# damaggu/StableKeypoints

Measured on AMD Instinct MI355X. Metric: images/sec (token-opt step, 512², N=500 tokens), higher is better.
Workload: dtype f32

## Files before the change

stablekeypoints_amd/csrc/skp_conv.hip:

```cpp
#include <cstdlib>
#include <initializer_list>
#include <type_traits>

#include "skp_common.h"
#include "skp_gn.h"

using namespace skp;

#ifndef SKP_WINO_DEBUG
#define SKP_WINO_DEBUG 0
#endif
#ifndef SKP_WINO2_DEBUG
#define SKP_WINO2_DEBUG 0
#endif

namespace {

typedef float f32x4 __attribute__((ext_vector_type(4)));
typedef unsigned int u32x4 __attribute__((ext_vector_type(4)));

constexpr int kMT = 64;
constexpr int kNC = 32;
constexpr int kCK = 4;
constexpr int kP = 36;
// ... 329 lines not shown
  if (!(a.nsplit == 1 || a.ws))
    return (form & kStride2) ? "split-K needs a workspace of nsplit·B·K·(H/2)·(W/2) floats"
                             : "split-K needs a workspace of nsplit·B·K·H·W floats";
  if (!a.aligned) return "tensors must be 16-byte aligned";
  if (!(form & kHW32) && (long long)a.B * (a.H / 4) * (a.W / 4) > 0x7fffffffLL - kMT) return "too many tiles";
  if ((form & kOffsets32) && !((long long)a.B * a.C * a.H * a.W * 4 < 0x7fffffffLL))
    return "input larger than 2 GiB (32-bit buffer offsets)";
  return nullptr;
}
constexpr long long kMaxGrid = 0x7fffffffLL;

}

extern "C" int skp_wino_weights(const float* w, int K, int C, int flip, float* U, void* stream) {
  const char* err = weights_args_error(w, U, K, C);
  SKP_CHECK_ARG(!err, err);
  const long long n = (long long)K * C;
  hipLaunchKernelGGL(wino_weights_kernel<kP>, dim3((unsigned)((n + 255) / 256)), dim3(256), 0, as_stream(stream), w, K,
                     C, flip, U);
  SKP_LAUNCH_CHECK();
  return SKP_OK;
}

namespace {

__global__ void splitk_reduce_kernel(const float4* __restrict__ ws, int nsplit, long long n4, int K, int hw4,
                                     const float* __restrict__ bias, const float4* __restrict__ res,
                                     float4* __restrict__ y) {
  const long long i = blockIdx.x * (long long)blockDim.x + threadIdx.x;
  if (i >= n4) return;
  float4 v = ws[i];
  for (int s = 1; s < nsplit; ++s) {
    const float4 p = ws[(long long)s * n4 + i];
    v.x += p.x;
    v.y += p.y;
    v.z += p.z;
    v.w += p.w;
  }
  if (bias) {
    const float b = bias[(i / hw4) % K];
    v.x += b;
    v.y += b;
    v.z += b;
    v.w += b;
  }
  if (res) {
    const float4 r = res[i];
    v.x += r.x;
    v.y += r.y;
    v.z += r.z;
    v.w += r.w;
  }
  y[i] = v;
}

int splitk_reduce(const float* ws, int nsplit, int B, int K, int HW, const float* bias, const float* residual,
                  float* y, hipStream_t st) {
  const long long n4 = (long long)B * K * HW / 4;
  hipLaunchKernelGGL(splitk_reduce_kernel, dim3((unsigned)((n4 + 255) / 256)), dim3(256), 0, st,
                     reinterpret_cast<const float4*>(ws), nsplit, n4, K, HW / 4, bias,
                     reinterpret_cast<const float4*>(residual), reinterpret_cast<float4*>(y));
  SKP_LAUNCH_CHECK();
  return SKP_OK;
}

int wino_nt_flag(long long out_bytes, int nsplit) {
  if (nsplit > 1) return 0;
  return out_bytes >= (256LL << 20) ? 128 : 0;
}

template <int NEPI, class F>
auto with_epi(int epi, F&& f) {
  static_assert(NEPI == 2 || NEPI == 4, "bias only, or bias and residual");
  if constexpr (NEPI == 4) {
    if (epi == 2) return f(std::integral_constant<int, 2>{});
    if (epi == 3) return f(std::integral_constant<int, 3>{});
  }
  return epi == 1 ? f(std::integral_constant<int, 1>{}) : f(std::integral_constant<int, 0>{});
}

template <class Launch>
int conv_launch(const char* entry, const float* bias, const float* residual, float* y, float* ws, int nsplit, int B, int K,
                int hw, int dbg, bool nt, hipStream_t st, Launch&& launch) {
  const int epi = nsplit > 1 ? 0 : (bias ? 1 : 0) | (residual ? 2 : 0);
  launch(epi, nsplit > 1 ? ws : y, dbg | (nt ? wino_nt_flag((long long)B * K * hw * 4, nsplit) : 0));
  const hipError_t e = hipGetLastError();
  if (e != hipSuccess) {
    set_error(std::string(entry) + ": launch failed: " + hipGetErrorString(e));
    return SKP_ELAUNCH;
  }
  if (nsplit > 1) return splitk_reduce(ws, nsplit, B, K, hw, bias, residual, y, st);
  return SKP_OK;
}

}

extern "C" int skp_conv3x3_wino(const float* x, const float* U, const float* bias, const float* residual, float* y,
                                int B, int C, int K, int H, int W, int nsplit, float* ws, void* stream) {
  const ConvArgs a{x && U && y, all_aligned16({x, U, y, residual, ws}), ws, nullptr, B, C, K, H, W, nsplit, 1};
  const char* err = conv_args_error(kOffsets32, a);
  const int tw = W / 4, tpi = (H / 4) * tw;
  const long long ntiles = (long long)B * tpi;
  const bool wide = ntiles <= 32 && K % 64 == 0;
  const int mt = wide ? 32 : kMT;
  const int ntb = (int)((ntiles + mt - 1) / mt), nkb = K / (wide ? 64 : kNC);
  if (!err && (long long)ntb * nkb * nsplit > kMaxGrid) err = "grid too large";
  SKP_CHECK_ARG(!err, err);
  const long long ubytes = (long long)K * C * kP * 4;
  const int kb_major = ubytes > (2LL << 20);
  hipStream_t st = as_stream(stream);
  const dim3 grid((unsigned)(ntb * nkb * nsplit));
  return conv_launch(__func__, bias, residual, y, ws, nsplit, B, K, H * W, SKP_WINO_DEBUG, false, st,
                     [&](int epi, float* out, int dbg) {
                       const auto kernel = with_epi<4>(
                           epi, [&](auto E) { return wide ? wino_f4_kernel<E(), 32> : wino_f4_kernel<E(), 64>; });
                       hipLaunchKernelGGL(kernel, grid, dim3(kThreads), 0, st, x, U, bias, residual, out, B, C, K, H, W, tw,
                                          tpi, (int)ntiles, ntb, nkb, kb_major, C / nsplit, dbg);
                     });
}

namespace {
namespace w2 {

constexpr int kNC = 32;
constexpr int kCK = 4;
constexpr int kNW = 4;
template <int TXB>
struct GeoN;
template <>
struct GeoN<8> {
  static constexpr int NI = 1, RR = 18, RC = 10, CHF = 768;
};
template <>
struct GeoN<4> {
  static constexpr int NI = 2, RR = 18, RC = 6, CHF = 880;
};
template <int TXB>
struct GeoT : GeoN<TXB> {
  using GeoN<TXB>::NI;
  using GeoN<TXB>::RR;
  using GeoN<TXB>::RC;
  using GeoN<TXB>::CHF;
  static constexpr int RF = 4 * RC;
  static constexpr int RAWF = (4 * CHF + 255) / 256 * 256;
  static constexpr int RAW_INSTR = RAWF / 256;
  static_assert(NI * RR * RF <= CHF, "channel region");
};
constexpr int kUP = 40;
constexpr int kUF = kCK * kNC * kUP;
constexpr int kUInstr = kUF / 256;
constexpr unsigned kOOB = 0x80000000u;
constexpr int kVWF = 4 * 256 + 128;
constexpr int kVF = 4 * kVWF;
constexpr int kUP2 = 28;
constexpr int kUF2 = kCK * kNC * kUP2;
typedef unsigned int u32x2 __attribute__((ext_vector_type(2)));
static_assert(kUF % 256 == 0 && kUF2 % 256 == 0, "whole 1-KB chunks");
static_assert((3 * GeoT<8>::RAWF + 2 * kUF) * 4 <= 80 * 1024 && 2 * (GeoT<4>::RAWF + kUF) * 4 <= 80 * 1024,
              "rings of two workgroups per CU");

__device__ constexpr float kAt[4][6] = {{1.f, 1.f, 1.f, 1.f, 1.f, 0.f},
                                        {0.f, 1.f, -1.f, 0.5f, -2.f, 0.f},
                                        {0.f, 1.f, 1.f, 0.25f, 4.f, 0.f},
                                        {0.f, 1.f, -1.f, 0.125f, -8.f, 1.f}};

#define W2_VMCNT(n) __builtin_amdgcn_s_waitcnt(((n) & 15) | (((n) >> 4) << 14) | (7 << 4) | (15 << 8))

typedef float f2 __attribute__((ext_vector_type(2)));

template <typename T>
__device__ __forceinline__ void bt6_shared(T a0, T a1, T a2, T a3, T a4, T a5, T* y) {
  const T e = a4 - a2, f = a3 - a1, g = a2 + a3, h = a3 - a2;
  y[0] = __builtin_elementwise_fma((T)1.5f, f, (a0 + e) - a2);
  y[1] = __builtin_elementwise_fma((T)1.5f, g, e + f);
  y[2] = __builtin_elementwise_fma((T)1.5f, h, e - f);
  y[3] = __builtin_elementwise_fma((T)2.0f, f, e);
  y[4] = __builtin_elementwise_fma((T)-0.5f, f, e);
  y[5] = __builtin_elementwise_fma((T)1.5f, e, __builtin_elementwise_fma((T)-2.0f, f, a5 - a1));
}

template <int H, int RF>
__device__ __forceinline__ void half_transform_pk(const float* raw, float* a) {
  f2 t[3][3];
  f2 k0[3], k1[3], k2[3], k3[3];
#pragma unroll
  for (int r = 0; r < 6; ++r) {
    if (H == 1 && r == 0) continue;
    const f32x4 c0 = *reinterpret_cast<const f32x4*>(raw + r * RF);
    const f32x4 c1 = *reinterpret_cast<const f32x4*>(raw + r * RF + 4);
    const f32x4 c2 = *reinterpret_cast<const f32x4*>(raw + r * RF + 8);
    const f2 d[3] = {__builtin_shufflevector(c1, c1, 0, 1), __builtin_shufflevector(c1, c1, 2, 3),
                     __builtin_shufflevector(c0, c2, 3, 4)};
#pragma unroll
    for (int p = 0; p < 3; ++p) {
      if (H == 0) {
        if (r == 0) k0[p] = d[p];
        if (r == 1) { k1[p] = d[p]; k0[p] = __builtin_elementwise_fma((f2)-1.5f, d[p], k0[p]); }
        if (r == 2) { k2[p] = d[p]; k3[p] = __builtin_elementwise_fma((f2)1.5f, d[p], -k1[p]); }
        if (r == 3) { k1[p] = __builtin_elementwise_fma((f2)1.5f, d[p], -k2[p]); k3[p] = k3[p] + d[p]; }
        if (r == 4) {
          const f2 sv = k1[p] + d[p];
          t[0][p] = k0[p] + (sv - k2[p]);
          t[1][p] = sv + k3[p];
          t[2][p] = sv - k3[p];
        }
      } else {
        if (r == 1) k0[p] = d[p];
        if (r == 2) k1[p] = d[p];
        if (r == 3) { k2[p] = d[p] - k0[p]; k3[p] = __builtin_elementwise_fma((f2)-2.0f, k2[p], -k0[p]); }
        if (r == 4) {
          const f2 e = d[p] - k1[p];
          t[0][p] = __builtin_elementwise_fma((f2)2.0f, k2[p], e);
          t[1][p] = __builtin_elementwise_fma((f2)-0.5f, k2[p], e);
          k3[p] = __builtin_elementwise_fma((f2)1.5f, e, k3[p]);
        }
        if (r == 5) t[2][p] = k3[p] + d[p];
      }
    }
    asm volatile("" ::"v"(c0.x), "v"(c0.y), "v"(c0.z), "v"(c2.y), "v"(c2.z), "v"(c2.w));
  }
  const f2 u0 = __builtin_shufflevector(t[0][2], t[1][2], 0, 2), u1 = __builtin_shufflevector(t[0][0], t[1][0], 0, 2);
  const f2 u2 = __builtin_shufflevector(t[0][0], t[1][0], 1, 3), u3 = __builtin_shufflevector(t[0][1], t[1][1], 0, 2);
  const f2 u4 = __builtin_shufflevector(t[0][1], t[1][1], 1, 3), u5 = __builtin_shufflevector(t[0][2], t[1][2], 1, 3);
  f2 y01[6];
  bt6_shared<f2>(u0, u1, u2, u3, u4, u5, y01);
  float y2[6];
  bt6_shared<float>(t[2][2].x, t[2][0].x, t[2][0].y, t[2][1].x, t[2][1].y, t[2][2].y, y2);
#pragma unroll
  for (int j = 0; j < 6; ++j) {
    a[j] = y01[j].x;
    a[6 + j] = y01[j].y;
    a[12 + j] = y2[j];
  }
}

template <int H>
__device__ __forceinline__ void half_output(const float* m, float* y) {
  float s[3][4];
#pragma unroll
  for (int ii = 0; ii < 3; ++ii) at6(m[6 * ii], m[6 * ii + 1], m[6 * ii + 2], m[6 * ii + 3], m[6 * ii + 4], m[6 * ii + 5], s[ii], 1);
#pragma unroll
  for (int r = 0; r < 4; ++r)
#pragma unroll
    for (int c = 0; c < 4; ++c) {
      float v = 0.0f;
      bool first = true;
#pragma unroll
      for (int ii = 0; ii < 3; ++ii) {
        const float a = kAt[r][3 * H + ii];
        if (a == 0.0f) continue;
        v = first ? ((a == 1.0f) ? s[ii][c] : a * s[ii][c]) : fmaf(a, s[ii][c], v);
        first = false;
      }
      y[4 * r + c] = v;
    }
}

template <int H, int RF>
__device__ __forceinline__ void s2_transform(const float* raw, float* a) {
  constexpr int NR = H ? 2 : 3;
  float d[NR][5];
#pragma unroll
  for (int i = 0; i < NR; ++i) {
    const float* rp = raw + (H ? 2 + 2 * i : 1 + 2 * i) * RF;
    const float4 c1 = *reinterpret_cast<const float4*>(rp + 4);
    const float4 c2 = *reinterpret_cast<const float4*>(rp + 8);
    d[i][0] = c1.x;
    d[i][1] = c1.y;
    d[i][2] = c1.z;
    d[i][3] = c1.w;
    d[i][4] = c2.x;
    asm volatile("" ::"v"(c2.y), "v"(c2.z), "v"(c2.w));
  }
#pragma unroll
  for (int ii = 0; ii < NR; ++ii) {
    float t[5];
#pragma unroll
    for (int b = 0; b < 5; ++b)
      t[b] = H ? d[ii][b] : ii == 0 ? d[0][b] - d[1][b] : ii == 1 ? d[1][b] : d[1][b] - d[2][b];
    a[5 * ii] = t[0] - t[2];
    a[5 * ii + 1] = t[2];
    a[5 * ii + 2] = t[2] - t[4];
    a[5 * ii + 3] = t[1];
    a[5 * ii + 4] = t[3];
  }
}

template <int H>
__device__ __forceinline__ void s2_output(const float* m, float* y) {
  constexpr int NR = H ? 2 : 3;
  float s[NR][2];
#pragma unroll
  for (int ii = 0; ii < NR; ++ii) {
    s[ii][0] = (m[5 * ii] + m[5 * ii + 1]) + m[5 * ii + 3];
    s[ii][1] = (m[5 * ii + 1] - m[5 * ii + 2]) + m[5 * ii + 4];
  }
#pragma unroll
  for (int c = 0; c < 2; ++c) {
    y[c] = H ? s[0][c] : s[0][c] + s[1][c];
    y[2 + c] = H ? s[1][c] : s[1][c] - s[NR - 1][c];
  }
}

}

struct W2Smem {
// ... 92 lines not shown
        const int q = ufirst + NW * m;
        __builtin_amdgcn_raw_ptr_buffer_load_lds(ru, (lds_ptr_t)(us_lds + 256 * q), 16, lane * 16, q * 1024, 0, 0);
      }
  };

  const int kc = lane >> 4;
  const int tx = lane & (TXB - 1);
  const int ty = TXB == 8 ? 2 * wm + ((lane >> 3) & 1) : (lane >> 2) & 3;
  const int roff = kc * kChF + (TXB == 8 ? 0 : wm * RR * kRowF) + 4 * ty * kRowF + 4 * tx;
  const int uoff = (kc * w2::kNC + (lane & 15)) * kUP + (S2 ? 16 : 20) * HH;

  f32x4 acc[2][NP];
#pragma unroll
  for (int b = 0; b < 2; ++b)
#pragma unroll
    for (int q = 0; q < NP; ++q) acc[b][q] = f32x4{0.f, 0.f, 0.f, 0.f};
  float a0[NP], a1[NP];

  auto mfmas = [&](const float* us, const float (&acur)[NP]) {
    constexpr int N4 = (NP + 1) / 4;
#pragma unroll
    for (int b = 0; b < 2; ++b) {
      const float* ub = us + uoff + b * 16 * kUP;
      float u[4 * N4 + 2];
#pragma unroll
      for (int j = 0; j < N4; ++j) {
        const float4 v = *reinterpret_cast<const float4*>(ub + 4 * j);
        u[4 * j] = v.x;
        u[4 * j + 1] = v.y;
        u[4 * j + 2] = v.z;
        u[4 * j + 3] = v.w;
      }
      if constexpr (NP % 4 == 2) {
        const float2 v2 = *reinterpret_cast<const float2*>(ub + 4 * N4);
        u[4 * N4] = v2.x;
        u[4 * N4 + 1] = v2.y;
      }
#pragma unroll
      for (int q = 0; q < NP; ++q) acc[b][q] = __builtin_amdgcn_mfma_f32_16x16x4f32(acur[q], u[q], acc[b][q], 0, 0, 0);
    }
  };
  auto transform = [&](const float* raw, float (&an)[NP]) {
    if constexpr (S2) w2::s2_transform<HH, kRowF>(raw + roff, an);
    else w2::half_transform_pk<HH, kRowF>(raw + roff, an);
  };

  if constexpr (VST) {
    using w2::kVF;
    using w2::kVWF;
    const int bw = W >> 5;
    const size_t tb = (size_t)img * ((H >> 4) * bw) + (size_t)(y0 >> 4) * bw + (x0 >> 5);
    const float* Vb = x + (tb * (size_t)(C / w2::kCK) + (size_t)(c0 / w2::kCK)) * kVF + wv * kVWF;
    asm volatile("" : "+s"(Vb));
    struct AReg {
      u32x4 c[4];
      w2::u32x2 d;
    };
    auto issue_vu = [&](int t, AReg& an, float* us_lds) {
      const bool ok = t < nst;
      const size_t tt = ok ? (size_t)t : 0;
      const __amdgpu_buffer_rsrc_t rv =
          __builtin_amdgcn_make_buffer_rsrc((void*)(Vb + tt * kVF), (short)0, ok ? kVWF * 4 : 0, 0x00020000);
      const __amdgpu_buffer_rsrc_t ru =
          __builtin_amdgcn_make_buffer_rsrc((void*)(Ub + tt * kUF), (short)0, ok ? kUF * 4 : 0, 0x00020000);
#pragma unroll
      for (int j = 0; j < 4; ++j) an.c[j] = __builtin_amdgcn_raw_buffer_load_b128(rv, lane * 16, j * 1024, 0);
      an.d = __builtin_amdgcn_raw_buffer_load_b64(rv, lane * 8, 4096, 0);
#pragma unroll
      for (int m = 0; m < w2::kUInstr / NW; ++m) {
        const int q = wv + NW * m;
        __builtin_amdgcn_raw_ptr_buffer_load_lds(ru, (lds_ptr_t)(us_lds + 256 * q), 16, lane * 16, q * 1024, 0, 0);
      }
    };
    static_assert(w2::kUInstr % NW == 0, "whole chunks per wave");
    constexpr int kPerStage = 5 + w2::kUInstr / NW;
    auto vstep = [&](int s, const AReg& ac, const float* Us, AReg& ai, float* Ui) {
      W2_VMCNT(kPerStage);
      asm volatile("" ::: "memory");
      __builtin_amdgcn_s_waitcnt(0xC07F);
      __builtin_amdgcn_s_barrier();
      asm volatile("" ::: "memory");
      asm volatile("" ::"v"(ac.c[0]), "v"(ac.c[1]), "v"(ac.c[2]), "v"(ac.c[3]), "v"(ac.d));
      issue_vu(s + 2, ai, Ui);
      __builtin_amdgcn_sched_barrier(0);
      if (s < nst) {
        float a[18];
#pragma unroll
        for (int j = 0; j < 4; ++j)
#pragma unroll
          for (int i = 0; i < 4; ++i) {
            const unsigned v = ac.c[j][i];
            a[4 * j + i] = __uint_as_float(v);
          }
        const unsigned d0 = ac.d[0], d1 = ac.d[1];
        a[16] = __uint_as_float(d0);
        a[17] = __uint_as_float(d1);
        mfmas(Us, a);
      }
    };
    AReg A0, A1, A2;
    issue_vu(0, A0, U0);
    asm volatile("" ::: "memory");
    __builtin_amdgcn_sched_barrier(0);
    issue_vu(1, A1, U1);
    for (int s0 = 0; s0 < nst; s0 += 3) {
      vstep(s0, A0, U0, A2, U2);
      vstep(s0 + 1, A1, U1, A0, U0);
      vstep(s0 + 2, A2, U2, A1, U1);
    }
  } else {
    issue_raw(0, R0);
    issue_u(0, U0);
    issue_raw(1, R1);
    if (RS == 3) issue_raw(2, R2);
    w2_vmcnt(nst > 1 ? allow_pro : 0);
    __syncthreads();
    transform(R0, a0);

    auto step = [&](int s, float* Rn, float* Us, float* Ri, float* Ui, const float (&acur)[NP], float (&anext)[NP]) {
      w2_vmcnt(s + 1 < nst ? allow_step : 0);
      __syncthreads();
      if (s + 1 < nst) issue_u(s + 1, Ui);
      issue_raw(s + RS, Ri);
      const bool tr = s + 1 < nst && !(dbg & 1);
      if (HH == 0) {
        if (tr) transform(Rn, anext);
        if (!(dbg & 2)) mfmas(Us, acur);
      } else {
        if (!(dbg & 2)) mfmas(Us, acur);
        if (tr) transform(Rn, anext);
      }
    };
    constexpr int PER = RS == 2 ? 2 : 6;
    float* const Rsl[4] = {R0, R1, R2, nullptr};
    float* const Usl[2] = {U0, U1};
    for (int s0 = 0; s0 < ((dbg & 16) ? 0 : nst); s0 += PER) {
      step(s0, Rsl[1], Usl[0], Rsl[0], Usl[1], a0, a1);
  #pragma unroll
      for (int j = 1; j < PER; ++j) {
        if (s0 + j < nst) {
          if ((j & 1) == 0) step(s0 + j, Rsl[(j + 1) % RS], Usl[j % 2], Rsl[j % RS], Usl[(j + 1) % 2], a0, a1);
          else step(s0 + j, Rsl[(j + 1) % RS], Usl[j % 2], Rsl[j % RS], Usl[(j + 1) % 2], a1, a0);
        }
      }
    }

  }

  W2_VMCNT(0);
  __syncthreads();
  if (dbg & 32) return;
  if constexpr (S2) {
    constexpr int PLS2 = 8 * 16 + 4;
    static_assert(16 * PLS2 <= Geo::RAWF, "stride-2 exchange planes fit one raw slot");
    const int Ho = H / 2, Wo = W / 2;
    float* pl = R0 + (lane & 15) * PLS2 + 2 * (2 * wm + (lane >> 5)) * 16 + 8 * ((lane >> 4) & 1);
#pragma unroll
    for (int blk = 0; blk < 2; ++blk) {
      float o[4][4];
#pragma unroll
      for (int r = 0; r < 4; ++r) {
        float m[NP];
#pragma unroll
        for (int q = 0; q < NP; ++q) m[q] = acc[blk][q][r];
        w2::s2_output<HH>(m, o[r]);
      }
      if (HH != blk) {
#pragma unroll
        for (int f = 0; f < 2; ++f)
#pragma unroll
          for (int h = 0; h < 2; ++h)
            *reinterpret_cast<float4*>(pl + f * 16 + 4 * h) =
                make_float4(o[2 * h][2 * f], o[2 * h][2 * f + 1], o[2 * h + 1][2 * f], o[2 * h + 1][2 * f + 1]);
      }
      __syncthreads();
      if (HH == blk) {
#pragma unroll
        for (int f = 0; f < 2; ++f)
#pragma unroll
          for (int h = 0; h < 2; ++h) {
            float4* d = reinterpret_cast<float4*>(pl + f * 16 + 4 * h);
            const float4 p = *d;
            *d = make_float4(o[2 * h][2 * f] + p.x, o[2 * h][2 * f + 1] + p.y, o[2 * h + 1][2 * f] + p.z,
                             o[2 * h + 1][2 * f + 1] + p.w);
          }
      }
      __syncthreads();
#pragma unroll
      for (int i = 0; i < 16 * 32 / NT; ++i) {
        const int idx = i * NT + tid;
        const int c = idx >> 5, row = (idx >> 2) & 7, c4 = idx & 3;
        const float4 p = *reinterpret_cast<const float4*>(R0 + c * PLS2 + row * 16 + 4 * c4);
        const int k = kb * w2::kNC + 16 * blk + c;
        const float bv = (EPI & 1) ? bias[k] : 0.0f;
        const size_t o4 = (((size_t)img * K + k) * Ho + y0 / 2 + row) * Wo + x0 / 2 + 4 * c4;
        const float4 v = make_float4(p.x + bv, p.y + bv, p.z + bv, p.w + bv);
        if (dbg & 128) __builtin_nontemporal_store(f32x4{v.x, v.y, v.z, v.w}, reinterpret_cast<f32x4*>(y + o4));
        else if (!(dbg & 64)) *reinterpret_cast<float4*>(y + o4) = v;
      }
      if (blk == 0) __syncthreads();
    }
  } else {
    constexpr int PH = 16;
    constexpr int PLS = (TXB == 8 ? PH * 32 : NI * 256) + 4;
    float* const P2 = RS == 2 ? U1 : R2;
    auto plane_of = [&](int c) -> float* {
      float* b = (c >> 2) == 0 ? R0 : (c >> 2) == 1 ? R1 : (c >> 2) == 2 ? P2 : U0;
      return b + (c & 3) * PLS + (c >> 2) * 16;
    };
    float* pl = plane_of(lane & 15);
    const int pbase = TXB == 8 ? (4 * (2 * wm + (lane >> 5))) * 32 + 4 * (4 * ((lane >> 4) & 1))
                               : wm * 256 + (4 * (lane >> 4)) * 16;
    constexpr int PW = TXB == 8 ? 32 : 16;
#pragma unroll
    for (int blk = 0; blk < 2; ++blk) {
      if (HH != blk) {
#pragma unroll
        for (int r = 0; r < 4; ++r) {
          float m[18], o[16];
#pragma unroll
          for (int q = 0; q < 18; ++q) m[q] = acc[blk][q][r];
          w2::half_output<HH>(m, o);
#pragma unroll
          for (int f = 0; f < 4; ++f)
            *reinterpret_cast<float4*>(pl + pbase + f * PW + 4 * r) =
                make_float4(o[4 * f], o[4 * f + 1], o[4 * f + 2], o[4 * f + 3]);
        }
      }
      __syncthreads();
      if (HH == blk) {
#pragma unroll
        for (int r = 0; r < 4; ++r) {
          float m[18], o[16];
#pragma unroll
          for (int q = 0; q < 18; ++q) m[q] = acc[blk][q][r];
          w2::half_output<HH>(m, o);
#pragma unroll
          for (int f = 0; f < 4; ++f) {
            float4* d = reinterpret_cast<float4*>(pl + pbase + f * PW + 4 * r);
            const float4 p = *d;
            *d = make_float4(o[4 * f] + p.x, o[4 * f + 1] + p.y, o[4 * f + 2] + p.z, o[4 * f + 3] + p.w);
          }
        }
      }
      __syncthreads();
      constexpr int PCF = TXB == 8 ? PH * 8 : NI * 64;
      constexpr int NIT = 16 * PCF / NT;
      static_assert(TXB != 8 || NIT == 8, "TXB 8: eight wave instructions per wave");
      float g1[4] = {0.f, 0.f, 0.f, 0.f}, g2[4] = {0.f, 0.f, 0.f, 0.f}, piv[4] = {0.f, 0.f, 0.f, 0.f};
#pragma unroll
      for (int i = 0; i < NIT; ++i) {
        const int idx = TXB == 8 ? (((tid >> 6) * NIT + i) << 6) + (tid & 63) : i * NT + tid;
        const int c = idx / PCF, q = idx % PCF;
        const float4 v0 = *reinterpret_cast<const float4*>(plane_of(c) + 4 * q);
        const int k = kb * w2::kNC + 16 * blk + c;
        const float bv = (EPI & 1) ? bias[k] : 0.0f;
        size_t o;
        if (TXB == 8) {
          const int row = q >> 3, c4 = q & 7;
          o = (((size_t)img * K + k) * H + y0 + row) * W + x0 + 4 * c4;
        } else {
          o = ((size_t)(img + (q >> 6)) * K + k) * 256 + 4 * (q & 63);
        }
        float4 v = make_float4(v0.x + bv, v0.y + bv, v0.z + bv, v0.w + bv);
        if (EPI & 2) {
          const float4 rv = *reinterpret_cast<const float4*>(res + o);
          v.x += rv.x;
          v.y += rv.y;
          v.z += rv.z;
          v.w += rv.w;
        }
        if (dbg & 128) __builtin_nontemporal_store(f32x4{v.x, v.y, v.z, v.w}, reinterpret_cast<f32x4*>(y + o));
        else if (!(dbg & 64)) *reinterpret_cast<float4*>(y + o) = v;
        if (TXB == 8 && gnp) {
          if ((i & 1) == 0) piv[i >> 1] = __builtin_bit_cast(float, __builtin_amdgcn_readfirstlane(__builtin_bit_cast(int, v.x)));
          const float p = piv[i >> 1];
          const float dx = v.x - p, dy = v.y - p, dz = v.z - p, dw = v.w - p;
          g1[i >> 1] += (dx + dy) + (dz + dw);
          g2[i >> 1] += (dx * dx + dy * dy) + (dz * dz + dw * dw);
        }
      }
      if (TXB == 8 && gnp) {
        float a[4] = {g1[0], g2[0], g1[1], g2[1]}, b[4] = {g1[2], g2[2], g1[3], g2[3]};
        float u[4];
#pragma unroll
        for (int j = 0; j < 4; ++j) {
          asm volatile("s_nop 1\n\tv_permlane32_swap_b32 %0, %1" : "+v"(a[j]), "+v"(b[j]));
          u[j] = a[j] + b[j];
        }
        float w[2];
#pragma unroll
        for (int j = 0; j < 2; ++j) {
          float x0 = u[j], x1 = u[j + 2];
          asm volatile("s_nop 1\n\tv_permlane16_swap_b32 %0, %1" : "+v"(x0), "+v"(x1));
          w[j] = x0 + x1;
        }
        const int lane = tid & 63;
        const bool hi = (lane & 8) != 0;
        const float keep = hi ? w[1] : w[0], send = hi ? w[0] : w[1];
        float x = keep + dpp_read<0x140>(send);
        x += dpp_read<0x141>(x);
        x += dpp_read<0x4E>(x);
        x += dpp_read<0xB1>(x);
        const float x2 = __shfl_xor(x, 8, 64);
        if ((lane & 15) == 0) {
          const int r = lane >> 4;
          const int J = (tid >> 6) * NIT + 2 * r;
          const int c = (J << 6) / PCF, piece = ((J << 6) % PCF) >> 6;
          const int k = kb * w2::kNC + 16 * blk + c;
          const int seg = ((y0 + 8 * piece) >> 4) * (W >> 5) + (x0 >> 5);
          const float p = r == 0 ? piv[0] : r == 1 ? piv[1] : r == 2 ? piv[2] : piv[3];
          constexpr float inv_n = 1.0f / 512.0f;
          gnp[((size_t)img * K + k) * (size_t)((H >> 4) * (W >> 5)) + seg] =
              make_float2(p + x * inv_n, fmaxf(x2 - x * (x * inv_n), 0.0f));
        }
      }
      if (blk == 0) __syncthreads();
    }
  }
}

template <int EPI, int TXB, bool S2 = false>
__global__ __launch_bounds__(w2::kNW * WAVE) __attribute__((amdgpu_waves_per_eu(2, 2))) void wino2_kernel(
    const float* __restrict__ x, const float* __restrict__ U, const float* __restrict__ bias,
    const float* __restrict__ res, float* __restrict__ y, int nimg, int C, int K, int H, int W, int bw, int bpi,
    int nblk, int nkb, int kb_major, int csplit, int dbg, float2* __restrict__ gnp) {
  constexpr int RAWF = w2::GeoT<TXB>::RAWF;
  __shared__ __attribute__((aligned(16))) float R0[RAWF], R1[RAWF], R2[TXB == 4 ? 4 : RAWF];
  constexpr int UF = S2 ? w2::kUF2 : w2::kUF;
  __shared__ __attribute__((aligned(16))) float U0[UF], U1[UF];
  const int G = gridDim.x;
  const int g = blockIdx.x;
  const int Lg = (G % 8 == 0) ? (g % 8) * (G / 8) + g / 8 : g;
  const int sp = Lg / (nblk * nkb);
  const int L = Lg - sp * (nblk * nkb);
  y += (size_t)sp * nimg * K * (S2 ? (H / 2) * (W / 2) : H * W);
  int tb, kb;
  if (kb_major) {
    kb = L / nblk;
    tb = L - kb * nblk;
  } else {
    tb = L / nkb;
    kb = L - tb * nkb;
  }
  int img, x0 = 0, y0 = 0;
  if (TXB == 8) {
    img = tb / bpi;
    const int br = tb - img * bpi;
    const int by = br / bw;
    x0 = 32 * (br - by * bw);
    y0 = 16 * by;
  } else {
    img = 2 * tb;
  }
  const int wv = __builtin_amdgcn_readfirstlane(threadIdx.x >> 6);
  const W2Smem sm{R0, R1, R2, U0, U1, nullptr};
  const int c0 = sp * csplit;
  if (wv < w2::kNW / 2)
    wino2_body<EPI, 0, TXB, false, S2>(sm, x, U, bias, res, y, C, K, H, W, img, x0, y0, kb, c0, csplit, wv, dbg, gnp);
  else wino2_body<EPI, 1, TXB, false, S2>(sm, x, U, bias, res, y, C, K, H, W, img, x0, y0, kb, c0, csplit, wv, dbg, gnp);
}

__global__ void wino2s2_weights_kernel(const float* __restrict__ w, int K, int C, float* __restrict__ U) {
  const long long i = blockIdx.x * (long long)blockDim.x + threadIdx.x;
  if (i >= (long long)K * C) return;
  const int k = (int)(i / C), c = (int)(i - (long long)k * C);
  double g[9];
  for (int u = 0; u < 9; ++u) g[u] = (double)w[((size_t)k * C + c) * 9 + u];
  const double Gm[5][3] = {{1.0, 0.0, 0.0}, {1.0, 0.0, 1.0}, {0.0, 0.0, 1.0}, {0.0, 1.0, 0.0}, {0.0, 1.0, 0.0}};
  double t[5][3];
  for (int a = 0; a < 5; ++a)
    for (int v = 0; v < 3; ++v) t[a][v] = Gm[a][0] * g[v] + Gm[a][1] * g[3 + v] + Gm[a][2] * g[6 + v];
  float* out = U + (((size_t)(k / w2::kNC) * C + c) * w2::kNC + (k % w2::kNC)) * w2::kUP2;
  for (int p = 0; p < w2::kUP2; ++p) out[p] = 0.0f;
  for (int a = 0; a < 5; ++a)
    for (int b = 0; b < 5; ++b) {
      const int p = 5 * a + b;
      out[p < 15 ? p : p + 1] = (float)(t[a][0] * Gm[b][0] + t[a][1] * Gm[b][1] + t[a][2] * Gm[b][2]);
    }
}

template <int EPI>
__global__ __launch_bounds__(w2::kNW * WAVE) __attribute__((amdgpu_waves_per_eu(2, 2))) void wino2v_kernel(
    const float* __restrict__ V, const float* __restrict__ U, const float* __restrict__ bias,
    const float* __restrict__ res, float* __restrict__ y, int nimg, int C, int K, int H, int W, int bw, int bpi,
    int nblk, int nkb, int kb_major, int csplit, int dbg, float2* __restrict__ gnp) {
  __shared__ __attribute__((aligned(16))) float U0[w2::kUF], U1[w2::kUF], U2[w2::kUF];
  static_assert(3 * w2::kUF * 4 <= 80 * 1024, "two workgroups per CU");
  static_assert(4 * (16 * 32 + 4) + 48 <= w2::kUF / 2, "a plane buffer per half U slot");
  const int G = gridDim.x;
  const int g = blockIdx.x;
  const int Lg = (G % 8 == 0) ? (g % 8) * (G / 8) + g / 8 : g;
  const int sp = Lg / (nblk * nkb);
  const int L = Lg - sp * (nblk * nkb);
  y += (size_t)sp * nimg * K * H * W;
  int tb, kb;
  if (kb_major) {
    kb = L / nblk;
    tb = L - kb * nblk;
  } else {
    tb = L / nkb;
    kb = L - tb * nkb;
  }
  const int img = tb / bpi;
  const int br = tb - img * bpi;
  const int by = br / bw;
  const int x0 = 32 * (br - by * bw), y0 = 16 * by;
  const int wv = __builtin_amdgcn_readfirstlane(threadIdx.x >> 6);
  const W2Smem sm{U0 + w2::kUF / 2, U1 + w2::kUF / 2, nullptr, U0, U1, U2};
  const int c0 = sp * csplit;
  if (wv < w2::kNW / 2)
    wino2_body<EPI, 0, 8, true>(sm, V, U, bias, res, y, C, K, H, W, img, x0, y0, kb, c0, csplit, wv, dbg, gnp);
  else wino2_body<EPI, 1, 8, true>(sm, V, U, bias, res, y, C, K, H, W, img, x0, y0, kb, c0, csplit, wv, dbg, gnp);
}

template <int GN>
__global__ __launch_bounds__(4 * WAVE) void wino2_vtransform_kernel(
    const float* __restrict__ x, const float* __restrict__ stats, const float* __restrict__ gamma,
    const float* __restrict__ beta, const float* __restrict__ shift, int G, float* __restrict__ V, int C, int H, int W,
    int bw, int bpi) {
  using Geo = w2::GeoT<8>;
  constexpr int RR = Geo::RR, RC = Geo::RC, kChF = Geo::CHF, kRowF = Geo::RF;
  __shared__ __attribute__((aligned(16))) float R[Geo::RAWF];
  const int tid = threadIdx.x, lane = tid & 63;
  const int nst = C / w2::kCK;
  const int tb = blockIdx.x / nst, st = blockIdx.x - tb * nst;
  const int img = tb / bpi;
  const int br = tb - img * bpi;
  const int by = br / bw;
  const int x0 = 32 * (br - by * bw), y0 = 16 * by;
  const int cpg = C / (G > 0 ? G : 1);
  for (int f = tid; f < w2::kCK * RR * RC; f += 4 * WAVE) {
    const int ch = f / (RR * RC), e = f - ch * (RR * RC);
    const int row = e / RC, c4 = e - row * RC;
    const int yy = y0 - 1 + row, xx = x0 - 4 + 4 * c4;
    float4 v = make_float4(0.f, 0.f, 0.f, 0.f);
    if (yy >= 0 && yy < H && xx >= 0 && xx < W) {
      const int c = w2::kCK * st + ch;
      v = *reinterpret_cast<const float4*>(x + (((size_t)img * C + c) * H + yy) * W + xx);
      if (GN) {
        const int grp = img * G + c / cpg;
        const GNCoef k = gn_coef(gamma[c], beta[c], stats[2 * grp], stats[2 * grp + 1]);
        const float t = shift ? shift[(size_t)img * C + c] : 0.0f;
        v.x = gn_elem<GN == 2>(v.x, t, k); v.y = gn_elem<GN == 2>(v.y, t, k);
        v.z = gn_elem<GN == 2>(v.z, t, k); v.w = gn_elem<GN == 2>(v.w, t, k);
      }
    }
    *reinterpret_cast<float4*>(R + ch * kChF + row * kRowF + 4 * c4) = v;
  }
  __syncthreads();
  const int wv = __builtin_amdgcn_readfirstlane(tid >> 6);
  const int HH = wv >> 1, wm = wv & 1;
  const int kc = lane >> 4, tx = lane & 7, ty = 2 * wm + ((lane >> 3) & 1);
  const int roff = kc * kChF + 4 * ty * kRowF + 4 * tx;
  float a[18];
  if (HH == 0) w2::half_transform_pk<0, kRowF>(R + roff, a);
  else w2::half_transform_pk<1, kRowF>(R + roff, a);
  float* o = V + (size_t)blockIdx.x * w2::kVF + wv * w2::kVWF;
#pragma unroll
  for (int j = 0; j < 4; ++j)
    *reinterpret_cast<float4*>(o + 256 * j + 4 * lane) = make_float4(a[4 * j], a[4 * j + 1], a[4 * j + 2], a[4 * j + 3]);
  *reinterpret_cast<float2*>(o + 1024 + 2 * lane) = make_float2(a[16], a[17]);
}

}

extern "C" int skp_wino2_weights(const float* w, int K, int C, int flip, float* U, void* stream) {
  const char* err = weights_args_error(w, U, K, C);
  SKP_CHECK_ARG(!err, err);
  const long long n = (long long)K * C;
  hipLaunchKernelGGL(wino_weights_kernel<w2::kUP>, dim3((unsigned)((n + 255) / 256)), dim3(256), 0, as_stream(stream), w,
                     K, C, flip, U);
  SKP_LAUNCH_CHECK();
  return SKP_OK;
}

extern "C" int skp_wino2s2_weights(const float* w, int K, int C, float* U, void* stream) {
  const char* err = weights_args_error(w, U, K, C);
  SKP_CHECK_ARG(!err, err);
  const long long n = (long long)K * C;
  hipLaunchKernelGGL(wino2s2_weights_kernel, dim3((unsigned)((n + 255) / 256)), dim3(256), 0, as_stream(stream), w, K,
                     C, U);
  SKP_LAUNCH_CHECK();
  return SKP_OK;
}

namespace {
using W2Kernel = void (*)(const float*, const float*, const float*, const float*, float*, int, int, int, int, int, int,
                          int, int, int, int, int, int, float2*);
template <int NEPI, class KernelOf>
int wino2_launch(const char* entry, KernelOf&& kernel_of, const float* x, const float* U, const float* bias,
                 const float* residual, float* y, int B, int C, int K, int H, int W, long long nblk, int hw, int nsplit,
                 float* ws, float* gn_part, void* stream) {
  const int bw = W / 32, bpi = (H / 16) * bw, nkb = K / w2::kNC;
  hipStream_t st = as_stream(stream);
  const dim3 grid((unsigned)(nblk * nkb * nsplit));
  return conv_launch(entry, bias, residual, y, ws, nsplit, B, K, hw, SKP_WINO2_DEBUG, true, st,
                     [&](int epi, float* out, int flags) {
                       const W2Kernel kernel = with_epi<NEPI>(epi, kernel_of);
                       hipLaunchKernelGGL(kernel, grid, dim3(w2::kNW * WAVE), 0, st, x, U, bias, residual, out, B, C, K, H,
                                          W, bw, bpi, (int)nblk, nkb, 0, C / nsplit, flags,
                                          reinterpret_cast<float2*>(gn_part));
                     });
}
}

extern "C" int skp_conv3x3s2_f2(const float* x, const float* U, const float* bias, float* y, int B, int C, int K,
                                int H, int W, int nsplit, float* ws, void* stream) {
  const ConvArgs a{x && U && y, all_aligned16({x, U, y, ws}), ws, nullptr, B, C, K, H, W, nsplit, 1};
  const char* err = conv_args_error(kHW32 | kStride2 | kOffsets32, a);
  const long long nblk = (long long)B * (H / 16) * (W / 32);
  if (!err && nblk * (K / w2::kNC) * nsplit > kMaxGrid) err = "grid too large";
  SKP_CHECK_ARG(!err, err);
  return wino2_launch<2>(
      __func__, [](auto E) -> W2Kernel { return wino2_kernel<E(), 8, true>; }, x, U, bias, nullptr, y, B, C, K, H, W, nblk,
      (H / 2) * (W / 2), nsplit, ws, nullptr, stream);
}

extern "C" int skp_conv3x3_wino2_gn(const float* x, const float* U, const float* bias, const float* residual, float* y,
                                    int B, int C, int K, int H, int W, int nsplit, float* ws, float* gn_part,
                                    void* stream) {
  const ConvArgs a{x && U && y, all_aligned16({x, U, y, residual, ws}), ws, gn_part, B, C, K, H, W, nsplit, 1};
  const char* err = conv_args_error(kHW32 | kOr16x16 | kOffsets32, a);
  const bool g16 = H == 16 && W == 16;
  const long long nblk = g16 ? B / 2 : (long long)B * (H / 16) * (W / 32);
  if (!err && nblk * (K / w2::kNC) * nsplit > kMaxGrid) err = "grid too large";
  SKP_CHECK_ARG(!err, err);
  return wino2_launch<4>(
      __func__, [g16](auto E) -> W2Kernel { return g16 ? wino2_kernel<E(), 4> : wino2_kernel<E(), 8>; }, x, U, bias,
      residual, y, B, C, K, H, W, nblk, H * W, nsplit, ws, gn_part, stream);
}

extern "C" int skp_conv3x3_wino2(const float* x, const float* U, const float* bias, const float* residual, float* y,
                                 int B, int C, int K, int H, int W, int nsplit, float* ws, void* stream) {
  return skp_conv3x3_wino2_gn(x, U, bias, residual, y, B, C, K, H, W, nsplit, ws, nullptr, stream);
}

namespace {
int vtransform_launch(const float* x, const float* stats, const float* gamma, const float* beta, const float* shift,
                      int G, int act, float* V, int B, int C, int H, int W, void* stream) {
  const int bw = W / 32, bpi = (H / 16) * bw;
  const long long nwg = (long long)B * bpi * (C / w2::kCK);
  if (nwg > kMaxGrid) return -2;
  const dim3 grid((unsigned)nwg), block(4 * WAVE);
  hipStream_t st = as_stream(stream);
  if (!stats) hipLaunchKernelGGL(wino2_vtransform_kernel<0>, grid, block, 0, st, x, stats, gamma, beta, shift, G, V, C, H, W, bw, bpi);
  else if (!act) hipLaunchKernelGGL(wino2_vtransform_kernel<1>, grid, block, 0, st, x, stats, gamma, beta, shift, G, V, C, H, W, bw, bpi);
  else hipLaunchKernelGGL(wino2_vtransform_kernel<2>, grid, block, 0, st, x, stats, gamma, beta, shift, G, V, C, H, W, bw, bpi);
  return 0;
}
}

extern "C" int skp_wino2_vtransform(const float* x, float* V, int B, int C, int H, int W, void* stream) {
  const ConvArgs a{x && V, all_aligned16({x, V}), nullptr, nullptr, B, C, w2::kNC, H, W, 1, 1};
  const char* err = conv_args_error(kHW32, a);
  if (!err && vtransform_launch(x, nullptr, nullptr, nullptr, nullptr, 0, 0, V, B, C, H, W, stream) != 0)
    err = "grid too large";
  SKP_CHECK_ARG(!err, err);
  SKP_LAUNCH_CHECK();
  return SKP_OK;
}

// ... 30 lines not shown
```

Baseline: 45.39.

## Merge two-block Winograd epilogue into single pass over all 32 output planes

The Winograd output epilogue used to exchange and store the two 16-channel blocks in two sequential passes, each with its own barriers. It now stages all 32 channel planes in shared memory at once: ring buffers R0-R2/U0-U1, or U0-U2 plus a new PT tail buffer in the V-staged kernel. That lets one exchange, one barrier sequence and one store pass cover the whole tile, and the stride-2 path gets the same treatment. Residual loads are hoisted ahead of the barrier, and group-norm partial reductions are regrouped per eight instructions. The cost is extra LDS for the V-staged kernel (PT) and more registers held for prefetched residuals.

After: 45.70 (median of 6 runs). No clear change (+0.7%).

```diff
diff --git a/stablekeypoints_amd/csrc/skp_conv.hip b/stablekeypoints_amd/csrc/skp_conv.hip
--- a/stablekeypoints_amd/csrc/skp_conv.hip
+++ b/stablekeypoints_amd/csrc/skp_conv.hip
@@ -505,6 +505,7 @@
 constexpr unsigned kOOB = 0x80000000u;
 constexpr int kVWF = 4 * 256 + 128;
 constexpr int kVF = 4 * kVWF;
+constexpr int kVPlaneF = 2688;
 constexpr int kUP2 = 28;
 constexpr int kUF2 = kCK * kNC * kUP2;
 typedef unsigned int u32x2 __attribute__((ext_vector_type(2)));
@@ -903,12 +904,10 @@
   if (dbg & 32) return;
   if constexpr (S2) {
     constexpr int PLS2 = 8 * 16 + 4;
-    static_assert(16 * PLS2 <= Geo::RAWF, "stride-2 exchange planes fit one raw slot");
+    static_assert(16 * PLS2 <= Geo::RAWF, "a block's stride-2 exchange planes fit one raw slot");
     const int Ho = H / 2, Wo = W / 2;
-    float* pl = R0 + (lane & 15) * PLS2 + 2 * (2 * wm + (lane >> 5)) * 16 + 8 * ((lane >> 4) & 1);
-#pragma unroll
-    for (int blk = 0; blk < 2; ++blk) {
-      float o[4][4];
+    const int poff = (lane & 15) * PLS2 + 2 * (2 * wm + (lane >> 5)) * 16 + 8 * ((lane >> 4) & 1);
+    auto tiles = [&](int blk, float (&o)[4][4]) {
 #pragma unroll
       for (int r = 0; r < 4; ++r) {
         float m[NP];
@@ -916,61 +915,82 @@
         for (int q = 0; q < NP; ++q) m[q] = acc[blk][q][r];
         w2::s2_output<HH>(m, o[r]);
       }
-      if (HH != blk) {
-#pragma unroll
-        for (int f = 0; f < 2; ++f)
-#pragma unroll
-          for (int h = 0; h < 2; ++h)
-            *reinterpret_cast<float4*>(pl + f * 16 + 4 * h) =
-                make_float4(o[2 * h][2 * f], o[2 * h][2 * f + 1], o[2 * h + 1][2 * f], o[2 * h + 1][2 * f + 1]);
-      }
-      __syncthreads();
-      if (HH == blk) {
-#pragma unroll
-        for (int f = 0; f < 2; ++f)
-#pragma unroll
-          for (int h = 0; h < 2; ++h) {
-            float4* d = reinterpret_cast<float4*>(pl + f * 16 + 4 * h);
-            const float4 p = *d;
-            *d = make_float4(o[2 * h][2 * f] + p.x, o[2 * h][2 * f + 1] + p.y, o[2 * h + 1][2 * f] + p.z,
-                             o[2 * h + 1][2 * f + 1] + p.w);
-          }
-      }
-      __syncthreads();
-#pragma unroll
-      for (int i = 0; i < 16 * 32 / NT; ++i) {
-        const int idx = i * NT + tid;
-        const int c = idx >> 5, row = (idx >> 2) & 7, c4 = idx & 3;
-        const float4 p = *reinterpret_cast<const float4*>(R0 + c * PLS2 + row * 16 + 4 * c4);
-        const int k = kb * w2::kNC + 16 * blk + c;
-        const float bv = (EPI & 1) ? bias[k] : 0.0f;
-        const size_t o4 = (((size_t)img * K + k) * Ho + y0 / 2 + row) * Wo + x0 / 2 + 4 * c4;
-        const float4 v = make_float4(p.x + bv, p.y + bv, p.z + bv, p.w + bv);
-        if (dbg & 128) __builtin_nontemporal_store(f32x4{v.x, v.y, v.z, v.w}, reinterpret_cast<f32x4*>(y + o4));
-        else if (!(dbg & 64)) *reinterpret_cast<float4*>(y + o4) = v;
-      }
-      if (blk == 0) __syncthreads();
+    };
+    {
+      float o[4][4];
+      tiles(1 - HH, o);
+      float* pl = (HH ? R0 : R1) + poff;
+#pragma unroll
+      for (int f = 0; f < 2; ++f)
+#pragma unroll
+        for (int h = 0; h < 2; ++h)
+          *reinterpret_cast<float4*>(pl + f * 16 + 4 * h) =
+              make_float4(o[2 * h][2 * f], o[2 * h][2 * f + 1], o[2 * h + 1][2 * f], o[2 * h + 1][2 * f + 1]);
+    }
+    __syncthreads();
+    {
+      float o[4][4];
+      tiles(HH, o);
+      float* pl = (HH ? R1 : R0) + poff;
+#pragma unroll
+      for (int f = 0; f < 2; ++f)
+#pragma unroll
+        for (int h = 0; h < 2; ++h) {
+          float4* d = reinterpret_cast<float4*>(pl + f * 16 + 4 * h);
+          const float4 p = *d;
+          *d = make_float4(o[2 * h][2 * f] + p.x, o[2 * h][2 * f + 1] + p.y, o[2 * h + 1][2 * f] + p.z,
+                           o[2 * h + 1][2 * f + 1] + p.w);
+        }
+    }
+    __syncthreads();
+#pragma unroll
+    for (int i = 0; i < 32 * 32 / NT; ++i) {
+      const int idx = i * NT + tid;
+      const int c = idx >> 5, row = (idx >> 2) & 7, c4 = idx & 3;
+      const float4 p = *reinterpret_cast<const float4*>((i < 2 ? R0 : R1) + (c & 15) * PLS2 + row * 16 + 4 * c4);
+      const int k = kb * w2::kNC + c;
+      const float bv = (EPI & 1) ? bias[k] : 0.0f;
+      const size_t o4 = (((size_t)img * K + k) * Ho + y0 / 2 + row) * Wo + x0 / 2 + 4 * c4;
+      const float4 v = make_float4(p.x + bv, p.y + bv, p.z + bv, p.w + bv);
+      if (dbg & 128) __builtin_nontemporal_store(f32x4{v.x, v.y, v.z, v.w}, reinterpret_cast<f32x4*>(y + o4));
+      else if (!(dbg & 64)) *reinterpret_cast<float4*>(y + o4) = v;
     }
   } else {
     constexpr int PH = 16;
+    int el = lane;
+    asm volatile("" : "+v"(el));
     constexpr int PLS = (TXB == 8 ? PH * 32 : NI * 256) + 4;
-    float* const P2 = RS == 2 ? U1 : R2;
-    auto plane_of = [&](int c) -> float* {
-      float* b = (c >> 2) == 0 ? R0 : (c >> 2) == 1 ? R1 : (c >> 2) == 2 ? P2 : U0;
-      return b + (c & 3) * PLS + (c >> 2) * 16;
+    constexpr bool ONEP = TXB == 8;
+    constexpr int NPASS = ONEP ? 1 : 2, CPP = w2::kNC / NPASS;
+    static_assert(!ONEP || VST || (40 + 5 * PLS <= Geo::RAWF && 60 + 9 * PLS <= w2::kUF), "32 planes in R0-R2, U0, U1");
+    static_assert(!VST || (36 + 9 * PLS <= w2::kUF && 44 + 5 * PLS <= w2::kVPlaneF), "32 planes in U0-U2 and the tail");
+    auto plane_of = [=](int c) -> float* {
+      if constexpr (!ONEP) {
+        float* b = (c >> 2) == 0 ? R0 : (c >> 2) == 1 ? R1 : (c >> 2) == 2 ? U1 : U0;
+        return b + (c & 3) * PLS + (c >> 2) * 16;
+      } else if constexpr (VST) {
+        const int f = c < 9 ? 0 : c < 18 ? 9 : c < 27 ? 18 : 27;
+        float* b = c < 9 ? U0 : c < 18 ? U1 : c < 27 ? U2 : R0;
+        return b + (c - f) * PLS + ((4 * f) & 63);
+      } else {
+        const int f = c < 5 ? 0 : c < 10 ? 5 : c < 15 ? 10 : c < 24 ? 15 : 24;
+        float* b = c < 5 ? R0 : c < 10 ? R1 : c < 15 ? R2 : c < 24 ? U0 : U1;
+        return b + (c - f) * PLS + ((4 * f) & 63);
+      }
     };
-    float* pl = plane_of(lane & 15);
-    const int pbase = TXB == 8 ? (4 * (2 * wm + (lane >> 5))) * 32 + 4 * (4 * ((lane >> 4) & 1))
-                               : wm * 256 + (4 * (lane >> 4)) * 16;
+    const int pbase = TXB == 8 ? (4 * (2 * wm + (el >> 5))) * 32 + 4 * (4 * ((el >> 4) & 1))
+                               : wm * 256 + (4 * (el >> 4)) * 16;
     constexpr int PW = TXB == 8 ? 32 : 16;
 #pragma unroll
-    for (int blk = 0; blk < 2; ++blk) {
-      if (HH != blk) {
+    for (int pass = 0; pass < NPASS; ++pass) {
+      if (ONEP || HH != pass) {
+        constexpr int OB = 1 - HH;
+        float* pl = plane_of((ONEP ? 16 * OB : 0) + (el & 15));
 #pragma unroll
         for (int r = 0; r < 4; ++r) {
           float m[18], o[16];
 #pragma unroll
-          for (int q = 0; q < 18; ++q) m[q] = acc[blk][q][r];
+          for (int q = 0; q < 18; ++q) m[q] = acc[OB][q][r];
           w2::half_output<HH>(m, o);
 #pragma unroll
           for (int f = 0; f < 4; ++f)
@@ -979,12 +999,13 @@
         }
       }
       __syncthreads();
-      if (HH == blk) {
+      if (ONEP || HH == pass) {
+        float* pl = plane_of((ONEP ? 16 * HH : 0) + (el & 15));
 #pragma unroll
         for (int r = 0; r < 4; ++r) {
           float m[18], o[16];
 #pragma unroll
-          for (int q = 0; q < 18; ++q) m[q] = acc[blk][q][r];
+          for (int q = 0; q < 18; ++q) m[q] = acc[HH][q][r];
           w2::half_output<HH>(m, o);
 #pragma unroll
           for (int f = 0; f < 4; ++f) {
@@ -994,79 +1015,88 @@
           }
         }
       }
+      constexpr int PCF = TXB == 8 ? PH * 8 : NI * 64;
+      constexpr int NIT = CPP * PCF / NT;
+      static_assert(TXB != 8 || NIT == 16, "TXB 8: sixteen wave instructions per wave");
+      static_assert(NIT % 8 == 0, "groups of eight wave instructions");
+      auto ch = [&](int i) { return TXB == 8 ? (wv * NIT + i) >> 1 : 2 * i + (wv >> 1); };
+      auto pf = [&](int i) { return 256 * (TXB == 8 ? i & 1 : wv & 1); };
+      const int k0 = kb * w2::kNC + CPP * pass + ch(0);
+      const size_t ub = TXB == 8 ? (((size_t)img * K + k0) * H + y0) * W + x0 : ((size_t)(img + (wv & 1)) * K + k0) * 256;
+      const unsigned vl = 4u * (unsigned)(TXB == 8 ? (el >> 3) * W + 4 * (el & 7) : 4 * el);
+      auto eoff = [&](int i) -> unsigned {
+        return vl + 4u * (unsigned)(TXB == 8 ? (i >> 1) * (H * W) + (i & 1) * 8 * W : 512 * i);
+      };
+      const char* const rp = reinterpret_cast<const char*>(res + ub);
+      char* const yp = reinterpret_cast<char*>(y + ub);
+      float4 rv[NIT];
+      if (EPI & 2) {
+#pragma unroll
+        for (int i = 0; i < NIT; ++i) rv[i] = *reinterpret_cast<const float4*>(rp + eoff(i));
+      }
       __syncthreads();
-      constexpr int PCF = TXB == 8 ? PH * 8 : NI * 64;
-      constexpr int NIT = 16 * PCF / NT;
-      static_assert(TXB != 8 || NIT == 8, "TXB 8: eight wave instructions per wave");
-      float g1[4] = {0.f, 0.f, 0.f, 0.f}, g2[4] = {0.f, 0.f, 0.f, 0.f}, piv[4] = {0.f, 0.f, 0.f, 0.f};
-#pragma unroll
-      for (int i = 0; i < NIT; ++i) {
-        const int idx = TXB == 8 ? (((tid >> 6) * NIT + i) << 6) + (tid & 63) : i * NT + tid;
-        const int c = idx / PCF, q = idx % PCF;
-        const float4 v0 = *reinterpret_cast<const float4*>(plane_of(c) + 4 * q);
-        const int k = kb * w2::kNC + 16 * blk + c;
-        const float bv = (EPI & 1) ? bias[k] : 0.0f;
-        size_t o;
-        if (TXB == 8) {
-          const int row = q >> 3, c4 = q & 7;
-          o = (((size_t)img * K + k) * H + y0 + row) * W + x0 + 4 * c4;
-        } else {
-          o = ((size_t)(img + (q >> 6)) * K + k) * 256 + 4 * (q & 63);
+#pragma unroll
+      for (int grp = 0; grp < NIT / 8; ++grp) {
+        float g1[4] = {0.f, 0.f, 0.f, 0.f}, g2[4] = {0.f, 0.f, 0.f, 0.f}, piv[4] = {0.f, 0.f, 0.f, 0.f};
+#pragma unroll
+        for (int j = 0; j < 8; ++j) {
+          const int i = 8 * grp + j;
+          const float4 v0 = *reinterpret_cast<const float4*>(plane_of(ch(i)) + pf(i) + 4 * el);
+          const float bv = (EPI & 1) ? bias[kb * w2::kNC + CPP * pass + ch(i)] : 0.0f;
+          float4 v = make_float4(v0.x + bv, v0.y + bv, v0.z + bv, v0.w + bv);
+          if (EPI & 2) {
+            v.x += rv[i].x;
+            v.y += rv[i].y;
+            v.z += rv[i].z;
+            v.w += rv[i].w;
+          }
+          if (dbg & 128) __builtin_nontemporal_store(f32x4{v.x, v.y, v.z, v.w}, reinterpret_cast<f32x4*>(yp + eoff(i)));
+          else if (!(dbg & 64)) *reinterpret_cast<float4*>(yp + eoff(i)) = v;
+          if (TXB == 8 && gnp) {
+            if ((j & 1) == 0) piv[j >> 1] = __builtin_bit_cast(float, __builtin_amdgcn_readfirstlane(__builtin_bit_cast(int, v.x)));
+            const float p = piv[j >> 1];
+            const float dx = v.x - p, dy = v.y - p, dz = v.z - p, dw = v.w - p;
+            g1[j >> 1] += (dx + dy) + (dz + dw);
+            g2[j >> 1] += (dx * dx + dy * dy) + (dz * dz + dw * dw);
+          }
         }
-        float4 v = make_float4(v0.x + bv, v0.y + bv, v0.z + bv, v0.w + bv);
-        if (EPI & 2) {
-          const float4 rv = *reinterpret_cast<const float4*>(res + o);
-          v.x += rv.x;
-          v.y += rv.y;
-          v.z += rv.z;
-          v.w += rv.w;
+        if (TXB == 8 && gnp) {
+          float a[4] = {g1[0], g2[0], g1[1], g2[1]}, b[4] = {g1[2], g2[2], g1[3], g2[3]};
+          float u[4];
+#pragma unroll
+          for (int j = 0; j < 4; ++j) {
+            asm volatile("s_nop 1\n\tv_permlane32_swap_b32 %0, %1" : "+v"(a[j]), "+v"(b[j]));
+            u[j] = a[j] + b[j];
+          }
+          float w[2];
+#pragma unroll
+          for (int j = 0; j < 2; ++j) {
+            float x0 = u[j], x1 = u[j + 2];
+            asm volatile("s_nop 1\n\tv_permlane16_swap_b32 %0, %1" : "+v"(x0), "+v"(x1));
+            w[j] = x0 + x1;
+          }
+          const int lane = tid & 63;
+          const bool hi = (lane & 8) != 0;
+          const float keep = hi ? w[1] : w[0], send = hi ? w[0] : w[1];
+          float x = keep + dpp_read<0x140>(send);
+          x += dpp_read<0x141>(x);
+          x += dpp_read<0x4E>(x);
+          x += dpp_read<0xB1>(x);
+          const float x2 = __shfl_xor(x, 8, 64);
+          if ((lane & 15) == 0) {
+            const int r = lane >> 4;
+            const int J = wv * NIT + 8 * grp + 2 * r;
+            const int c = (J << 6) / PCF, piece = ((J << 6) % PCF) >> 6;
+            const int k = kb * w2::kNC + CPP * pass + c;
+            const int seg = ((y0 + 8 * piece) >> 4) * (W >> 5) + (x0 >> 5);
+            const float p = r == 0 ? piv[0] : r == 1 ? piv[1] : r == 2 ? piv[2] : piv[3];
+            constexpr float inv_n = 1.0f / 512.0f;
+            gnp[((size_t)img * K + k) * (size_t)((H >> 4) * (W >> 5)) + seg] =
+                make_float2(p + x * inv_n, fmaxf(x2 - x * (x * inv_n), 0.0f));
+          }
         }
-        if (dbg & 128) __builtin_nontemporal_store(f32x4{v.x, v.y, v.z, v.w}, reinterpret_cast<f32x4*>(y + o));
-        else if (!(dbg & 64)) *reinterpret_cast<float4*>(y + o) = v;
-        if (TXB == 8 && gnp) {
-          if ((i & 1) == 0) piv[i >> 1] = __builtin_bit_cast(float, __builtin_amdgcn_readfirstlane(__builtin_bit_cast(int, v.x)));
-          const float p = piv[i >> 1];
-          const float dx = v.x - p, dy = v.y - p, dz = v.z - p, dw = v.w - p;
-          g1[i >> 1] += (dx + dy) + (dz + dw);
-          g2[i >> 1] += (dx * dx + dy * dy) + (dz * dz + dw * dw);
-        }
-      }
-      if (TXB == 8 && gnp) {
-        float a[4] = {g1[0], g2[0], g1[1], g2[1]}, b[4] = {g1[2], g2[2], g1[3], g2[3]};
-        float u[4];
-#pragma unroll
-        for (int j = 0; j < 4; ++j) {
-          asm volatile("s_nop 1\n\tv_permlane32_swap_b32 %0, %1" : "+v"(a[j]), "+v"(b[j]));
-          u[j] = a[j] + b[j];
-        }
-        float w[2];
-#pragma unroll
-        for (int j = 0; j < 2; ++j) {
-          float x0 = u[j], x1 = u[j + 2];
-          asm volatile("s_nop 1\n\tv_permlane16_swap_b32 %0, %1" : "+v"(x0), "+v"(x1));
-          w[j] = x0 + x1;
-        }
-        const int lane = tid & 63;
-        const bool hi = (lane & 8) != 0;
-        const float keep = hi ? w[1] : w[0], send = hi ? w[0] : w[1];
-        float x = keep + dpp_read<0x140>(send);
-        x += dpp_read<0x141>(x);
-        x += dpp_read<0x4E>(x);
-        x += dpp_read<0xB1>(x);
-        const float x2 = __shfl_xor(x, 8, 64);
-        if ((lane & 15) == 0) {
-          const int r = lane >> 4;
-          const int J = (tid >> 6) * NIT + 2 * r;
-          const int c = (J << 6) / PCF, piece = ((J << 6) % PCF) >> 6;
-          const int k = kb * w2::kNC + 16 * blk + c;
-          const int seg = ((y0 + 8 * piece) >> 4) * (W >> 5) + (x0 >> 5);
-          const float p = r == 0 ? piv[0] : r == 1 ? piv[1] : r == 2 ? piv[2] : piv[3];
-          constexpr float inv_n = 1.0f / 512.0f;
-          gnp[((size_t)img * K + k) * (size_t)((H >> 4) * (W >> 5)) + seg] =
-              make_float2(p + x * inv_n, fmaxf(x2 - x * (x * inv_n), 0.0f));
-        }
-      }
-      if (blk == 0) __syncthreads();
+      }
+      if (pass + 1 < NPASS) __syncthreads();
     }
   }
 }
@@ -1137,8 +1167,8 @@
     const float* __restrict__ res, float* __restrict__ y, int nimg, int C, int K, int H, int W, int bw, int bpi,
     int nblk, int nkb, int kb_major, int csplit, int dbg, float2* __restrict__ gnp) {
   __shared__ __attribute__((aligned(16))) float U0[w2::kUF], U1[w2::kUF], U2[w2::kUF];
-  static_assert(3 * w2::kUF * 4 <= 80 * 1024, "two workgroups per CU");
-  static_assert(4 * (16 * 32 + 4) + 48 <= w2::kUF / 2, "a plane buffer per half U slot");
+  __shared__ __attribute__((aligned(16))) float PT[w2::kVPlaneF];
+  static_assert(2 * (3 * w2::kUF + w2::kVPlaneF) * 4 <= 160 * 1024, "two workgroups per CU");
   const int G = gridDim.x;
   const int g = blockIdx.x;
   const int Lg = (G % 8 == 0) ? (g % 8) * (G / 8) + g / 8 : g;
@@ -1158,7 +1188,7 @@
   const int by = br / bw;
   const int x0 = 32 * (br - by * bw), y0 = 16 * by;
   const int wv = __builtin_amdgcn_readfirstlane(threadIdx.x >> 6);
-  const W2Smem sm{U0 + w2::kUF / 2, U1 + w2::kUF / 2, nullptr, U0, U1, U2};
+  const W2Smem sm{PT, nullptr, nullptr, U0, U1, U2};
   const int c0 = sp * csplit;
   if (wv < w2::kNW / 2)
     wino2_body<EPI, 0, 8, true>(sm, V, U, bias, res, y, C, K, H, W, img, x0, y0, kb, c0, csplit, wv, dbg, gnp);
```
